# davidfischinger/haf_grasping

Hardware: AMD Instinct MI355X
Metric: grid-cell x rotation SVM evals/sec (higher is better)
Workload: dtype f16

## Files before the change

### haf_grasping_amd/build.py

```python
import os
import re
import subprocess
import sys

HERE = os.path.dirname(os.path.abspath(__file__))
CSRC = os.path.join(HERE, "csrc")
LIB = os.path.join(HERE, "libhafgrasp.so")
LIB_TESTING = os.path.join(HERE, "libhafgrasp_testing.so")
ENGINE_SOURCES = ["engine.cpp", "engine_tables.cpp", "engine_request.cpp", "engine_geometry.cpp", "engine_debug.cpp", "engine_topgrasps.cpp", "engine_graspmap.cpp", "engine_roi.cpp", "engine_depthfilter.cpp", "engine_segment.cpp", "engine_cellsegment.cpp", "engine_plane.cpp", "engine_clearance.cpp", "engine_opening.cpp", "engine_space.cpp", "engine_labelshape.cpp", "engine_objects.cpp", "engine_transfer.cpp", "engine_stage.cpp"]
TESTING_ONLY = ["engine_testing.cpp", "testkernels.hip"]
SOURCES = ["prestages.hip", "features.hip", "contraction.hip", "screen.hip", "recheck.hip", "exact8.hip", "vote.hip", "prob.hip", "topgrasps.hip", "frames.hip", "graspmap.hip", "roi.hip", "depthfilter.hip", "segment.hip", "cellsegment.hip", "plane.hip", "clearance.hip", "opening.hip", "space.hip", "labelshape.hip", "transfer.hip"] + \
          ENGINE_SOURCES + ["parsers.cpp", "model_tables.cpp", "frames_host.cpp", "frame_stage.cpp", "graspmap_host.cpp", "roi_host.cpp", "depthfilter_host.cpp", "segment_host.cpp", "cellsegment_host.cpp", "plane_host.cpp", "clearance_host.cpp", "opening_host.cpp", "space_host.cpp", "labelshape_host.cpp", "transfer_host.cpp", "multi.cpp"]
EXTRA = {"screen.hip": ["-fno-slp-vectorize"]}
HEADERS = ["kernels.h", "device_common.h", "feature_device.h", "screen_band.h", "screen_finish.h", "parsers.h", "model_tables.h", "decq.h", "engine_internal.h", "engine_state.h", "frame_points.h", "frames.h", "frame_stage.h", "frame_group.h", "object_group.h", "label_group.h", "grasp_cells.h", "pick_rules.h", "depth_filter.h", "segment_rules.h", "cell_segment_rules.h", "wave_union.h", "plane_rules.h", "clearance_rules.h", "opening_rules.h", "space_rules.h", "grasp_lane.h", "label_shape.h", "transfer_rules.h"] + TESTING_ONLY + [ os.path.join("..", "..", "include", "hafgrasp.h"),
           os.path.join("..", "cli", "haf_grasp_cli.cpp"), os.path.join("..", "..", "ros_shim", "shim_core.h")]
FLAGS = ["--offload-arch=gfx950", "-O3", "-std=c++17", "-fPIC", "-ffp-contract=off", "-fno-fast-math",
         "-Wall", "-Wno-unused-result", "-Wno-inline-asm"]
ROCM = os.environ.get("ROCM_PATH", "/opt/rocm")
OBJDUMP = os.path.join(ROCM, "lib", "llvm", "bin", "llvm-objdump")
EXP_HAZARD_KERNELS = ["k_svm_screen", "k_svm_rbf_h", "k_svm_rbf"]
EXP_MIN_DISTANCE = 8


def up_to_date():
    if not (os.path.exists(LIB) and os.path.exists(LIB_TESTING)):
        return False
    t = min(os.path.getmtime(LIB), os.path.getmtime(LIB_TESTING))
    deps = [os.path.join(CSRC, f) for f in SOURCES + HEADERS] + [os.path.abspath(__file__)]
    return all(os.path.getmtime(d) <= t for d in deps if os.path.exists(d))
# ... 310 lines not shown

def _compile_and_link(out_lib, out_testing, obj_dir, extra_flags=(), verbose=False, checks=True):
    hipcc = os.environ.get("HIPCC", os.path.join(ROCM, "bin", "hipcc"))
    os.makedirs(obj_dir, exist_ok=True)

    def compile_one(src, suffix="", defs=()):
        obj = os.path.join(obj_dir, os.path.splitext(src)[0] + suffix + ".o")
        cmd = [hipcc] + FLAGS + EXTRA.get(src, []) + os.environ.get("HAF_EXPERIMENT_FLAGS", "").split() + list(extra_flags) + list(defs) + \
              ["-c", os.path.join(CSRC, src), "-o", obj]
        if verbose:
            print(" ".join(cmd))
        subprocess.check_call(cmd)
        return obj

    from concurrent.futures import ThreadPoolExecutor
    jobs = [(src, "", ()) for src in SOURCES] + [(src, "_testing", ("-DHAF_TESTING",)) for src in ENGINE_SOURCES + TESTING_ONLY]
    with ThreadPoolExecutor(max_workers=max(1, int(os.environ.get("HAF_BUILD_JOBS", "4")))) as pool:
        done = list(pool.map(lambda j: compile_one(*j), jobs))
    objs = dict(zip(SOURCES, done[:len(SOURCES)]))
    testing_objs = dict(zip(ENGINE_SOURCES + TESTING_ONLY, done[len(SOURCES):]))
    link = [hipcc, "--offload-arch=gfx950", "-shared", "-fPIC"]
    libs = ["-L" + os.path.join(ROCM, "lib"), "-lrccl", "-lpthread", "-Wl,-rpath," + os.path.join(ROCM, "lib")]
    staged = []
    try:
        for out in (out_lib, out_testing):
            tmp = out + ".unchecked"
            if out == out_lib:
                members = [objs[s] for s in SOURCES]
            else:
                members = [testing_objs.get(s, objs[s]) for s in SOURCES] + [testing_objs[s] for s in TESTING_ONLY]
            cmd = link + members + libs + ["-o", tmp]
            if verbose:
                print(" ".join(cmd))
            subprocess.check_call(cmd)
            staged.append((tmp, out))
# ... 46 lines not shown
```

### haf_grasping_amd/capi.py

```python
import ctypes as C
import os

import numpy as np

HERE = os.path.dirname(os.path.abspath(__file__))
LIB_PATH = os.environ.get("HAF_LIB", os.path.join(HERE, "libhafgrasp.so"))
TESTLIB_PATH = os.environ.get("HAF_TESTLIB", os.path.join(HERE, "libhafgrasp_testing.so"))

HAF_OK, HAF_E_ARG, HAF_E_IO, HAF_E_DEVICE, HAF_E_CAPACITY, HAF_E_BUDGET, HAF_E_INTERNAL = 0, -1, -2, -3, -4, -5, -6
FLAG_KEEP_DEBUG, FLAG_PROFILE, FLAG_FP32_MFMA, FLAG_SPLIT_F16, FLAG_PROBABILITY, FLAG_FULL_RANK = 1, 2, 4, 8, 16, 32
DBG_HEIGHTS, DBG_INTEGRAL, DBG_MASK, DBG_LABELS, DBG_DECISION, DBG_TRANSFORM, DBG_SCREEN_MARGIN, DBG_PROBABILITY, DBG_GRASPSGRID, DBG_ROI = range(10)
SHARD_ROLLS, SHARD_CLOUDS = 0, 1
FRAME_DEPTH_U16, FRAME_DEPTH_F32, FRAME_XYZ_F32 = 0, 1, 2
MAP_NO_CELL = -32768
MAX_LABELS = 4096
STAGES = ["upload", "bin", "integral", "mask", "features", "svm", "refine", "recheck", "vote", "download"]


class Config(C.Structure):
    _fields_ = [("feature_file", C.c_char_p), ("range_file", C.c_char_p), ("model_file", C.c_char_p),
                ("nr_features_without_shaf", C.c_int32), ("grid_h", C.c_int32), ("grid_w", C.c_int32),
                ("n_rolls", C.c_int32), ("roll_step_deg", C.c_int32), ("z_shift", C.c_float),
                ("graspval_top", C.c_int32), ("device", C.c_int32), ("max_clouds", C.c_int32),
                ("max_points", C.c_int64), ("flags", C.c_uint32), ("graspval_th", C.c_int32),
# ... 354 lines not shown
    if testing:
        L.haf_test_decq_host.restype = C.c_double
        L.haf_test_decq_host.argtypes = [C.c_double, C.c_int]
        L.haf_test_scale_host.restype = C.c_double
        L.haf_test_scale_host.argtypes = [C.c_double] * 5
        L.haf_test_sigma_upper.restype = C.c_double
        L.haf_test_sigma_upper.argtypes = [C.c_void_p, C.c_int, C.c_int]
        L.haf_test_table_digest.argtypes = [E, C.c_char_p, C.c_int]
        L.haf_test_host_table_digest.argtypes = [C.POINTER(Config), C.c_double, C.c_double, C.c_char_p, C.c_int, C.c_char_p, C.c_int]
        L.haf_test_decq4_scr.restype = C.c_double
        L.haf_test_decq4_scr.argtypes = [C.c_float]
        L.haf_test_decq4_scr_n.argtypes = [C.c_void_p, C.c_void_p, C.c_int]
        L.haf_test_host_slot_table.argtypes = [C.POINTER(Config), C.c_double, C.c_double, C.c_int] + [C.c_void_p] * 8 + \
            [C.POINTER(C.c_int), C.c_char_p, C.c_int]
        L.haf_test_feature_thresholds.argtypes = [C.c_void_p]
        L.haf_test_feature_form.argtypes = [E, C.c_void_p, C.c_void_p, C.c_void_p, C.c_int, C.POINTER(C.c_int)]
        L.haf_test_screen_finish.argtypes = [E, C.c_void_p, C.c_int, C.c_void_p, C.c_void_p]
        L.haf_test_split3.restype = C.c_double
        L.haf_test_split3.argtypes = [C.c_double, C.c_void_p]
        L.haf_test_decq_device.argtypes = [C.c_void_p, C.c_void_p, C.c_int, C.c_int]
        L.haf_test_mfma_accum.argtypes = [C.c_void_p, C.c_void_p, C.c_void_p, C.c_void_p, C.c_int]
        L.haf_test_mfma_rate.argtypes = [C.c_int, C.c_int, C.POINTER(C.c_double)]
        L.haf_test_mfma_model.argtypes = [C.c_int, C.c_int, C.c_int, C.POINTER(C.c_double)]
        L.haf_test_scale_device.argtypes = [C.c_void_p, C.c_void_p, C.c_void_p, C.c_double, C.c_double, C.c_void_p,
                                            C.c_int]
        L.haf_test_feature_table.argtypes = [C.c_char_p, C.POINTER(C.c_int), C.c_void_p, C.c_void_p, C.c_int]
        L.haf_test_range_table.argtypes = [C.c_char_p, C.POINTER(C.c_double), C.POINTER(C.c_double),
                                           C.POINTER(C.c_int), C.c_void_p, C.c_void_p, C.c_void_p, C.c_int]
        L.haf_test_model.argtypes = [C.c_char_p, C.POINTER(C.c_double), C.POINTER(C.c_double), C.POINTER(C.c_int),
                                     C.POINTER(C.c_int), C.c_void_p, C.c_void_p, C.c_void_p, C.c_void_p, C.c_long]
# ... 1215 lines not shown
```

### haf_grasping_amd/csrc/engine_request.cpp

```cpp
#include "engine_state.h"

namespace haf_host {

static double host_kernel_value(const SvmModel &m, const double *xg, int n, int kx)
{
    double acc = 0.0;
    if (m.kernel_type == HAF_KERNEL_RBF) {
        for (int k = 0; k < kx; k++) {
            const double sv = k < m.dim ? m.sv[(size_t)n * m.dim + k] : 0.0;
            const double dd = xg[(size_t)k * 16] - sv;
            acc += dd * dd;
        }
        return std::exp(-m.gamma * acc);
    }
    for (int k = 0; k < kx; k++) {
        const double sv = k < m.dim ? m.sv[(size_t)n * m.dim + k] : 0.0;
        acc += xg[(size_t)k * 16] * sv;
    }
    if (m.kernel_type == HAF_KERNEL_POLY) {
        double tmp = m.gamma * acc + m.coef0, ret = 1.0;
        for (int t = m.degree; t > 0; t /= 2) { if (t % 2 == 1) ret *= tmp; tmp = tmp * tmp; }
        return ret;
    }
    if (m.kernel_type == HAF_KERNEL_SIGMOID) return std::tanh(m.gamma * acc + m.coef0);
// ... 589 lines not shown

static void fp64_window(haf_engine *e, const Request &q, const TierPlan &p, int off)
{
    if (p.fp64 == FP64_SMALL)
        launch_small_direct(e->d_ii.p, e->d_evalcell.p, e->d_counters.p, e->mdl.fd.p, e->mdl.sv64.p, e->mdl.exact, q.d, e->flag_cap, e->d_dec_exact.p,
                            e->d_labels.p, list_buf(e, p.fp64_out), e->list_cap, nullptr, q.s, list_buf(e, p.fp64_in), list_counter(p.fp64_in), off);
    else
        launch_recheck_mfma(e->d_ii.p, e->d_evalcell.p, e->mdl.fd.p, e->mdl.sv64.p, e->mdl.exact, list_buf(e, p.fp64_in), e->flag_cap, off, e->d_counters.p,
                            e->d_x64.p, e->d_part64.p, p.i8 ? e->d_dec_exacti.p : e->d_dec_exact.p, e->d_labels.p, list_buf(e, p.fp64_out), e->list_cap,
                            q.d, q.s, nullptr, false, list_counter(p.fp64_in), e->d_tier_words.p);
}
static void i8_window(haf_engine *e, const Request &q, const TierPlan &p, int off)
{
    launch_recheck_i8(e->d_ii.p, e->d_evalcell.p, e->mdl.fd.p, e->mdl.sv_i8.p, e->mdl.i8, e->range.lower, e->range.upper, list_buf(e, p.i8_in), e->flag_cap,
                      off, e->d_counters.p, e->d_x64.p, e->d_part64.p, e->d_dec_exact.p, e->d_labels.p, list_buf(e, p.i8_out), e->list_cap, q.d, q.s,
                      e->d_tier_words.p);
}

static int vote_and_wait(haf_engine *e, const Request &q)
{
    const hipStream_t s = q.s;
    mark(e, HAF_ST_VOTE);
    if (q.from.roi)
        launch_vote_roi(e->d_labels.p, reinterpret_cast<const float *>(e->d_heights.p), e->d_brcount.p, e->d_ev16.p, e->d_topkey.p, e->d_rowmax.p,
                        e->d_rec.p, e->d_roi_cells.p, q.d, s);
    else
        launch_vote(e->d_labels.p, reinterpret_cast<const float *>(e->d_heights.p), e->d_brcount.p, e->d_ev16.p, e->d_topkey.p, e->d_rowmax.p, e->d_rec.p, q.d, s);
    mark(e, HAF_ST_DOWNLOAD);
    HIPCHK(e, hipMemcpyAsync(e->out_block.host, e->out_block.dev.p, kCntBytes + (size_t)q.B * q.R * sizeof(RollRecordDev), hipMemcpyDeviceToHost, s));
    mark(e, HAF_ST_COUNT);
    if (q.short_request) {
// ... 298 lines not shown
```

### haf_grasping_amd/csrc/engine_tables.cpp

```cpp
#include "engine_state.h"

namespace haf_host {

TableSwitches table_switches()
{
    TableSwitches s;
    s.no_cr = test_env("HAF_NO_CR") != nullptr;
    s.no_lr = test_env("HAF_NO_LR") != nullptr;
    s.cr_no_centre = test_env("HAF_CR_NO_CENTRE") != nullptr;
    s.no_cr_t1 = test_env("HAF_NO_CR_T1") != nullptr;
    s.no_i8 = test_env("HAF_NO_I8") != nullptr;
    s.no_fast_groups = test_env("HAF_NO_FAST_GROUPS") != nullptr;
    s.screen_no_centre = test_env("HAF_SCREEN_NO_CENTRE") != nullptr;
    s.lr_unfused = test_env("HAF_LR_UNFUSED") != nullptr;
    s.no_lr_plain = test_env("HAF_NO_LR_PLAIN") != nullptr;
    s.kappa_t1_measured = test_env("HAF_KAPPA_T1_MEASURED") != nullptr;
    s.prob_host_all = test_env("HAF_PROB_HOST_ALL") != nullptr;
    s.host_exp_all = test_env("HAF_HOST_EXP_ALL") != nullptr;
    if (const char *g = test_env("HAF_GUARD_REL")) { s.guard_rel_set = true; s.guard_rel = guard_knob(g); }
    if (const char *g = test_env("HAF_GUARD0_REL")) { s.guard0_rel_set = true; s.guard0_rel = guard_knob(g); }
    if (const char *g = test_env("HAF_GUARD2_REL")) { s.guard2_rel_set = true; s.guard2_rel = guard_knob(g); }
    if (const char *g = test_env("HAF_GUARD_I8_REL")) { s.guard_i8_rel_set = true; s.guard_i8_rel = guard_knob(g); }
    return s;
}

static TableInputs table_inputs(const haf_engine *e)
{
    TableInputs in;
    in.cfg = e->cfg;
// ... 158 lines not shown
```

### haf_grasping_amd/csrc/engine_testing.cpp

```cpp
#include "engine_state.h"
#include "screen_finish.h"
#include "screen_band.h"

#ifndef HAF_TESTING
#error "engine_testing.cpp belongs to the testing build (-DHAF_TESTING)"
#endif

namespace haf_host {
namespace {
struct CanaryRec { char *user; size_t bytes; const char *file; int line; };
std::mutex g_canary_mu;
std::vector<CanaryRec> g_canary;
}
void canary_register(void *user, size_t bytes, const char *file, int line)
{
    std::lock_guard<std::mutex> lk(g_canary_mu);
    g_canary.push_back(CanaryRec{static_cast<char *>(user), bytes, file, line});
}
void canary_unregister(void *user)
{
    std::lock_guard<std::mutex> lk(g_canary_mu);
    for (size_t i = 0; i < g_canary.size(); i++)
        if (g_canary[i].user == user) { g_canary[i] = g_canary.back(); g_canary.pop_back(); return; }
}
// ... 597 lines not shown
                lr_finish_band(r, lb, o[0], o[1], o[2], o[3]);
            }
        }
        return (int)HAF_OK;
    });
    return rc == HAF_E_INTERNAL ? say(rc) : rc;
}

int haf_test_feature_thresholds(long long *out3)
{
    if (!out3) return HAF_E_ARG;
    out3[0] = kSmallEvals; out3[1] = kWaves16Evals; out3[2] = kLargeEvals;
    return HAF_OK;
}

int haf_test_feature_form(haf_engine *e, int *form, int *flags, unsigned long long *iiabs, int cap, int *n)
{
    if (!e || !form) return HAF_E_ARG;
    form[0] = e->feature_form; form[1] = e->feature_sp_kind; form[2] = e->feature_sp.cr_poly;
    const int br = e->last.B * e->last.R;
    if (n) *n = br;
    if (!flags && !iiabs) return HAF_OK;
    if (br <= 0 || br > cap) return HAF_E_ARG;
    if (hipDeviceSynchronize() != hipSuccess) return HAF_E_DEVICE;
    if (flags && (!e->d_inexact.p || (size_t)br > e->d_inexact.n ||
                  hipMemcpy(flags, e->d_inexact.p, (size_t)br * sizeof(int), hipMemcpyDeviceToHost) != hipSuccess)) return HAF_E_DEVICE;
    if (iiabs && (!e->d_iiabs.p || (size_t)br > e->d_iiabs.n ||
                  hipMemcpy(iiabs, e->d_iiabs.p, (size_t)br * sizeof(unsigned long long), hipMemcpyDeviceToHost) != hipSuccess)) return HAF_E_DEVICE;
    return HAF_OK;
}
// ... 224 lines not shown
```

### haf_grasping_amd/csrc/exact8.hip

```cpp
#include "device_common.h"

namespace haf {

typedef int i32x4 __attribute__((ext_vector_type(4)));

constexpr int kI8Waves = 4;
constexpr int kI8Evals = 16 * kI8Waves;
constexpr int kI8Split = 8;
static_assert(kRecheckPartRows == 2 * kI8Split + 1, "part64 layout shared with the fp64 tier");
constexpr int kI8TileLoads = kI8GroupBytes / (256 * 16);
static_assert(kI8TileLoads * 256 * 16 == kI8GroupBytes, "tile image = whole 16-byte loads of 256 threads");

__device__ __forceinline__ int window_count8(int total, int off, int cap) { return max(0, min(total - off, cap)); }

__device__ __forceinline__ double exp2_poly(double y)
{
    const double n = rint(y);
    const double f = y - n;
    double p = 4.4455382718708101e-10;
    p = fma(p, f, 7.0549116208011209e-09);
    p = fma(p, f, 1.0178086009239696e-07);
    p = fma(p, f, 1.3215486790144305e-06);
    p = fma(p, f, 1.5252733804059838e-05);
    p = fma(p, f, 0.00015403530393381606);
    p = fma(p, f, 0.0013333558146428441);
    p = fma(p, f, 0.0096181291076284769);
    p = fma(p, f, 0.055504108664821576);
    p = fma(p, f, 0.24022650695910069);
    p = fma(p, f, 0.69314718055994529);
    p = fma(p, f, 1.0);
    return ldexp(p, (int)fmax(n, -1200.0));
}

__device__ __forceinline__ void i8_tile_mfma(const char *bt, int lane, const i32x4 (&a)[kI8Slices][kI8Steps], i32x4 (&acc)[5])
{
#pragma unroll
    for (int w = 0; w < 5; w++) acc[w] = i32x4{0, 0, 0, 0};
    i32x4 b[kI8Slices], bn[kI8Slices];
#pragma unroll
    for (int k = 0; k < kI8Slices; k++) b[k] = *reinterpret_cast<const i32x4 *>(bt + (k * kI8Steps) * 1024 + lane * 16);
#pragma unroll
    for (int ks = 0; ks < kI8Steps; ks++) {
        if (ks + 1 < kI8Steps) {
#pragma unroll
            for (int k = 0; k < kI8Slices; k++) bn[k] = *reinterpret_cast<const i32x4 *>(bt + (k * kI8Steps + ks + 1) * 1024 + lane * 16);
        }
#define HAF_I8_MFMA(j, k) acc[(j) + (k)] = __builtin_amdgcn_mfma_i32_16x16x64_i8(a[j][ks], b[k], acc[(j) + (k)], 0, 0, 0)
        HAF_I8_MFMA(0, 3); HAF_I8_MFMA(1, 3); HAF_I8_MFMA(0, 2); HAF_I8_MFMA(1, 2); HAF_I8_MFMA(0, 1); HAF_I8_MFMA(2, 2); HAF_I8_MFMA(2, 1);
        HAF_I8_MFMA(1, 1); HAF_I8_MFMA(0, 0); HAF_I8_MFMA(3, 0); HAF_I8_MFMA(3, 1); HAF_I8_MFMA(2, 0); HAF_I8_MFMA(1, 0);
#undef HAF_I8_MFMA
#pragma unroll
        for (int k = 0; k < kI8Slices; k++) b[k] = bn[k];
    }
}

__device__ __forceinline__ void i8_tile_epilogue(const i32x4 (&acc)[5], const double (&xx)[4], double ss, double cf, double gamma2, double dq_scale,
                                                 double (&part)[4], double (&pabs)[4])
{
#pragma unroll
    for (int r = 0; r < 4; r++) {
        const int u1 = (acc[1][r] << 7) + acc[2][r], u2 = (acc[3][r] << 7) + acc[4][r];
        const double dq = fma(fma((double)acc[0][r], 16384.0, (double)u1), 16384.0, (double)u2);
        const double d2 = fma(dq_scale, dq, xx[r] + ss);
        const double kv = exp2_poly(-gamma2 * d2);
        part[r] = fma(cf, kv, part[r]);
        pabs[r] = fma(fabs(cf), kv, pabs[r]);
    }
}

__device__ __forceinline__ void i8_split(int n_flag, int flag_cap, int n_tiles, int &splits, size_t &pitch)
{
    const bool fine = (long)n_flag * 4 <= (long)flag_cap && n_tiles >= 16 * kI8Split && flag_cap >= 4 && n_flag <= 1024;
    const int n_groups = (n_flag + kI8Evals - 1) / kI8Evals;
    splits = fine ? max(kI8Split, min(4 * kI8Split, 512 / max(n_groups, 1))) : kI8Split;
    pitch = fine ? (size_t)(flag_cap / 4) : (size_t)flag_cap;
}

__global__ __launch_bounds__(256, 2) void k_recheck_i8(const char *__restrict__ ximg, const char *__restrict__ svimg, I8Params p,
                                                       int flag_cap, int list_off, const int *__restrict__ counters, int cslot,
                                                       double *__restrict__ part64)
{
    __shared__ __attribute__((aligned(16))) char bt[kI8SvTileBytes];
    const int n_flag = window_count8(counters[cslot], list_off, flag_cap);
    const int n_groups = (n_flag + kI8Evals - 1) / kI8Evals;
    const int tid = threadIdx.x, wave = tid >> 6, lane = tid & 63;
    const int n_tiles = p.n_sv_pad / 16;
    int splits;
    size_t pitch;
    i8_split(n_flag, flag_cap, n_tiles, splits, pitch);
    const int tiles_per_part = (n_tiles + splits - 1) / splits;
    const double *xnorm = part64 + (size_t)(2 * kI8Split) * flag_cap;
    for (int task = blockIdx.x; task < n_groups * splits; task += gridDim.x) {
        const int g = task / splits, h = task - g * splits;
// ... 83 lines not shown
            v += __shfl_xor(v, 1, 64); w += __shfl_xor(w, 1, 64);
            part[r] = v; pabs[r] = w;
        }
        if ((lane & 15) == 0) {
#pragma unroll
            for (int r = 0; r < 4; r++) {
                const int sl = grp * 16 + 4 * (lane >> 4) + r;
                if (sl < n_flag) {
                    part64[(size_t)(2 * h) * pitch + sl] = part[r];
                    part64[(size_t)(2 * h + 1) * pitch + sl] = pabs[r];
                }
            }
        }
    }
}

__global__ __launch_bounds__(256) void k_recheck_i8_combine(const double *__restrict__ part64, const int *__restrict__ evalcell, I8Params p,
                                                            const int *__restrict__ flag_list, int flag_cap, int list_off,
                                                            int *__restrict__ counters, int cslot, double *__restrict__ dec_exact,
                                                            int8_t *__restrict__ labels, int *__restrict__ flagi_list, int flagi_cap,
                                                            unsigned long long *__restrict__ words)
{
    const int n_flag = window_count8(counters[cslot], list_off, flag_cap);
    const int lane = threadIdx.x & 63;
    int splits;
    size_t pitch;
    i8_split(n_flag, flag_cap, p.n_sv_pad / 16, splits, pitch);
    for (int base = blockIdx.x * 256 + (threadIdx.x & ~63); base < n_flag; base += gridDim.x * 256) {
        const int sl = base + lane;
        bool undecided = false;
// ... 25 lines not shown
            if (lane == 0) words[base >> 6] = bal;
        }
    }
}

__global__ __launch_bounds__(kListCompactThreads) void k_i8_handover(const unsigned long long *__restrict__ words, const int *__restrict__ flag_list,
                                                                     int flag_cap, int list_off, int *__restrict__ counters, int cslot,
                                                                     int *__restrict__ flagi_list, int flagi_cap)
{
    __shared__ int s_scan[kListCompactThreads];
    list_compact_body(words, window_count8(counters[cslot], list_off, flag_cap), flag_list, flagi_list, flagi_cap, counters, CNT_FLAGGEDI, s_scan);
}

void launch_recheck_i8(const float *ii, const int *evalcell, const FeatDesc *fd, const void *sv_i8, I8Params p, double lower, double upper,
                       const int *flag_list, int window_cap, int list_off, int *counters, void *ximg, double *part64, double *dec_exact,
                       int8_t *labels, int *flagi_list, int flagi_cap, Dims d, hipStream_t s, unsigned long long *words)
{
    const int groups = (window_cap + kI8Evals - 1) / kI8Evals;
    if (groups <= 0) return;
    flag_list += list_off;
    dec_exact += list_off;
    launch_features(ii, evalcell, counters, fd, reinterpret_cast<float *>(ximg), reinterpret_cast<float *>(part64 + (size_t)(2 * kI8Split) * window_cap),
                    d, lower, upper, 0.0f, window_cap, XMODE_I8, ScreenParams{}, flag_list, CNT_FLAGGED, window_cap, false, window_cap, nullptr,
                    nullptr, s, list_off);
    const long tasks = (long)groups * 4 * kI8Split;
    hipLaunchKernelGGL(k_recheck_i8, dim3((unsigned)(tasks < 8192 ? tasks : 8192)), dim3(256), 0, s, (const char *)ximg, (const char *)sv_i8, p,
                       window_cap, list_off, counters, CNT_FLAGGED, part64);
    const int blocks = groups < 2048 ? groups : 2048;
    hipLaunchKernelGGL(k_recheck_i8_combine, dim3(blocks), dim3(256), 0, s, part64, evalcell, p, flag_list, window_cap, list_off, counters,
                       CNT_FLAGGED, dec_exact, labels, flagi_list, flagi_cap, words);
    if (words) hipLaunchKernelGGL(k_i8_handover, dim3(1), dim3(kListCompactThreads), 0, s, words, flag_list, window_cap, list_off, counters, CNT_FLAGGED,
                                  flagi_list, flagi_cap);
}

}
```

### haf_grasping_amd/csrc/kernels.h

```cpp
#pragma once

#include <hip/hip_runtime.h>
#include <stddef.h>
#include <stdint.h>
#include "frame_points.h"
#include "frames.h"
#include "grasp_cells.h"
#include "pick_rules.h"

namespace haf {

constexpr int kKP = 324;
constexpr int kKSteps = kKP / 2;
constexpr int kDP = 328;
constexpr int kTile = 32;
constexpr int kTileFloats = kDP * kTile;
constexpr int kSvmBlockEvals = 256;
constexpr int kSvmThreads = 512;
constexpr int kHListParts = 4;

constexpr int kHK = 336;
constexpr int kHFull = 10;
constexpr int kHSteps = kHK / 16;
constexpr int kHMatBytes = kHSteps * 1024;
// ... 211 lines not shown
enum { CNT_EVALS = 0, CNT_FLAGGED = 1, CNT_ERROR = 2, CNT_FLAGGED2 = 3, CNT_FLAGGED0 = 4,
       CNT_INEXACT = 5,
       CNT_FLAGGEDI = 6,
       CNT_FLAGGED0B = 7,
       CNT_BYPASS = 8,
       CNT_T1_N = 9,
       CNT_T1_ADD = 10,
       CNT_COUNT = 12 };

constexpr int kI8Q = 23;
constexpr long kI8Max = 63L * (2097152L + 16384L + 128L + 1L);
constexpr int kI8Slices = 4;
constexpr int kI8Steps = 6;
constexpr int kI8GroupBytes = kI8Slices * kI8Steps * 1024;
constexpr int kI8SvTileBytes = kI8GroupBytes + 256;
struct I8Params {
    double gamma, rho;
    double gamma2;
    double drop;
    double delta;
    double dq_scale;
    double s_max;
    double guard_scale;
    int n_sv_pad, gv0, gv1, pad;
};
void launch_recheck_i8(const float *ii, const int *evalcell, const FeatDesc *fd, const void *sv_i8, I8Params p, double lower, double upper,
                       const int *flag_list, int window_cap, int list_off, int *counters, void *ximg, double *part64, double *dec_exact,
                       int8_t *labels, int *flagi_list, int flagi_cap, Dims d, hipStream_t s,
                       unsigned long long *words = nullptr);

constexpr int kM64Rows = 326;

struct RollRecordDev { int vote; short row, col; float h_locmax; int n_evals; };

struct ProbParams {
    double A, B;
    int gv0, gv1;
    float hdr;
    int host_all;
    double dec_slack;
};
void launch_probability_eval(const double *dec_exact, const int *evalcell, const int *counters, ProbParams P, int8_t *labels, float *own,
                             double *ptext, int *near_list, int near_cap, int *counters_rw, long evals_cap, hipStream_t s);
void launch_prob_list(int *counters, int slot, int *list, int cap, hipStream_t s);
// ... 286 lines not shown
```

### haf_grasping_amd/csrc/model_tables.cpp

```cpp
#include "model_tables.h"

#include <algorithm>
#include <cmath>
#include <cstdio>
#include <cstdlib>
#include <cstring>

namespace haf_host {

float header_grid_value(int label0, int label1)
{
    char line[96];
    snprintf(line, sizeof line, "labels %d %d", label0, label1);
    const std::string ln(line);
    const int res = (int)atof(ln.substr(0, 2).c_str());
    int start = (int)ln.find(" ", 0), end = (int)ln.find(" ", (size_t)start + 1);
    if (res > 0) { start = end; end = (int)ln.find(" ", (size_t)start + 1); }
    const float prob = (float)atof(ln.substr((size_t)start, (size_t)end).c_str());
    return res * prob;
}

int label_grid_value(int label)
{
    char buf[32];
// ... 1031 lines not shown
        sv64[(size_t)kKP * t.n_sv_pad + n] = ss;
        sv64[(size_t)(kKP + 1) * t.n_sv_pad + n] = m.coef[(size_t)n];
        coef64[(size_t)n] = m.coef[(size_t)n];
        ss_max = std::max(ss_max, ss);
    }
    return ss_max;
}

void int8_planes(Work &w)
{
    const haf_config &c = w.in.cfg;
    const SvmModel &m = *w.in.model;
    const TableSwitches &sw = w.in.sw;
    ModelTables &t = w.t;
    t.i8_active = !(c.flags & HAF_FLAG_PROBABILITY) && !sw.no_i8 && t.kx <= 64 * kI8Steps && !w.in.generic_kernel;
    if (!t.i8_active) return;
    const int n_tiles16 = t.n_sv_pad / 16;
    std::vector<char> img((size_t)n_tiles16 * kI8SvTileBytes, 0);
    double s_max2 = 0.0;
    double sv_abs_max = 0.0;
    for (int n = 0; n < m.n_sv; n++)
        for (int k = 0; k < m.dim; k++) sv_abs_max = std::max(sv_abs_max, std::fabs(m.sv[(size_t)n * m.dim + k]));
    int qs = kI8Q;
    while (qs < 30 && (sv_abs_max * std::ldexp(1.0, qs + 1) + 1.0) <= (double)kI8Max) qs++;
    if (!(sv_abs_max < 1e30)) t.i8_active = false;
    for (int n = 0; n < m.n_sv && t.i8_active; n++) {
        char *tile = img.data() + (size_t)(n / 16) * kI8SvTileBytes;
        const int col = n % 16;
        long long ssq = 0;
        for (int k = 0; k < m.dim; k++) {
// ... 132 lines not shown
```

### haf_grasping_amd/csrc/model_tables.h

```cpp
#pragma once
#include "../../include/hafgrasp.h"
#include "kernels.h"
#include "parsers.h"

#include <string>
#include <vector>

using namespace haf;

namespace haf_host {

enum { MODE_SCREEN = 0, MODE_SPLIT = 1, MODE_F32 = 2 };
inline int contraction_mode(const haf_config &c)
{
    if (c.flags & HAF_FLAG_FP32_MFMA) return MODE_F32;
    if (c.flags & HAF_FLAG_SPLIT_F16) return MODE_SPLIT;
    return MODE_SCREEN;
}

struct TableSwitches {
    bool no_cr = false;
    bool no_lr = false;
    bool cr_no_centre = false;
    bool no_cr_t1 = false;
    bool no_i8 = false;
    bool no_fast_groups = false;
    bool screen_no_centre = false;
    bool lr_unfused = false;
    bool no_lr_plain = false;
    bool kappa_t1_measured = false;
    bool prob_host_all = false;
    bool host_exp_all = false;
    bool guard_rel_set = false, guard0_rel_set = false, guard2_rel_set = false, guard_i8_rel_set = false;
    double guard_rel = 1.0, guard0_rel = 1.0, guard2_rel = 1.0, guard_i8_rel = 1.0;
};

struct TableInputs {
    haf_config cfg{};
    const std::vector<FeatureRow> *features = nullptr;
    const RangeTable *range = nullptr;
    const SvmModel *model = nullptr;
    double mfma_kappa = 12.0, mfma_kappa16 = 12.0;
    bool generic_kernel = false;
// ... 47 lines not shown
    I8Params i8{};
    ProbParams prob{};

    int nf = 0, kx = 0, n_sv_tiles = 0, sv_tile_neg = 0, n_sv_pad = 0;
    double sum_abs_coef = 0;
    bool screen_active = true;
    bool cr_available = false;
    bool lr_available = false;
    bool lr_fused = true;
    bool lr_plain_available = false;
    bool t1_cr_available = false, i8_active = false;
    int lr_rank = 0;
    int gv0 = 0, gv1 = 0;
    bool prob_mode = false;
    double host_exp_thr = 0.0;
};

template <class T> using HostBuf = std::vector<T>;
struct ModelTables : TableSet<HostBuf>, ModelConsts {
    std::vector<int> slot_rep;
    std::vector<double> slot_mu;
};

struct TableError {
    int code = HAF_OK;
    std::string msg;
};

TableError build_model_tables(const TableInputs &in, ModelTables &t);

// ... 6 lines not shown
```

### haf_grasping_amd/csrc/screen.hip

```cpp
#include "kernels.h"
#include "screen_band.h"
#include <algorithm>
#include <cmath>
#include <vector>

namespace haf {

typedef float f32x4 __attribute__((ext_vector_type(4)));
typedef _Float16 half8 __attribute__((ext_vector_type(8)));
typedef _Float16 half4 __attribute__((ext_vector_type(4)));

__device__ __forceinline__ void dma_piece(const char *gbase, unsigned lds_dst, unsigned lane16)
{
    asm volatile("s_mov_b32 m0, %0\n\ts_nop 0\n\tglobal_load_lds_dwordx4 %1, %2" ::"s"(lds_dst), "v"(lane16), "s"(gbase) : "memory", "m0");
}

struct TileDma {
    const char *g[kS0WavePieces];
    unsigned l[kS0WavePieces];
};
__device__ __forceinline__ TileDma tile_dma(const char *gtile, unsigned lds_slot, const int (&poff)[kS0WavePieces])
{
    TileDma d;
#pragma unroll
    for (int q = 0; q < kS0WavePieces; q++) { d.g[q] = gtile + poff[q]; d.l[q] = lds_slot + (unsigned)poff[q]; }
    return d;
}
__device__ __forceinline__ void stage_sv_tile_s0(const TileDma &d, unsigned lane16)
{
    asm volatile("s_nop 4");
// ... 1127 lines not shown
```

Baseline: 535.3 million.

## Pipeline int8 recheck kernel with LDS DMA ring and interleaved epilogue

Rewrites the exact int8 recheck kernel so support-vector tiles are streamed into an LDS ring buffer through direct global-to-LDS loads. Each tile's MFMA sequence is interleaved with the DMA issues for the next tile and with the previous tile's double-precision exp epilogue, using sched barriers. The goal is to hide global load latency and epilogue ALU time behind matrix work. The old staged kernel is kept only as a testing-build option, and the grid cap becomes configurable, at the cost of more LDS per workgroup and more complex scheduling.

```diff
diff --git a/haf_grasping_amd/build.py b/haf_grasping_amd/build.py
--- a/haf_grasping_amd/build.py
+++ b/haf_grasping_amd/build.py
@@ -9,10 +9,11 @@
 LIB_TESTING = os.path.join(HERE, "libhafgrasp_testing.so")
 ENGINE_SOURCES = ["engine.cpp", "engine_tables.cpp", "engine_request.cpp", "engine_geometry.cpp", "engine_debug.cpp", "engine_topgrasps.cpp", "engine_graspmap.cpp", "engine_roi.cpp", "engine_depthfilter.cpp", "engine_segment.cpp", "engine_cellsegment.cpp", "engine_plane.cpp", "engine_clearance.cpp", "engine_opening.cpp", "engine_space.cpp", "engine_labelshape.cpp", "engine_objects.cpp", "engine_transfer.cpp", "engine_stage.cpp"]
 TESTING_ONLY = ["engine_testing.cpp", "testkernels.hip"]
+TESTING_KERNELS = ["exact8.hip"]
 SOURCES = ["prestages.hip", "features.hip", "contraction.hip", "screen.hip", "recheck.hip", "exact8.hip", "vote.hip", "prob.hip", "topgrasps.hip", "frames.hip", "graspmap.hip", "roi.hip", "depthfilter.hip", "segment.hip", "cellsegment.hip", "plane.hip", "clearance.hip", "opening.hip", "space.hip", "labelshape.hip", "transfer.hip"] + \
           ENGINE_SOURCES + ["parsers.cpp", "model_tables.cpp", "frames_host.cpp", "frame_stage.cpp", "graspmap_host.cpp", "roi_host.cpp", "depthfilter_host.cpp", "segment_host.cpp", "cellsegment_host.cpp", "plane_host.cpp", "clearance_host.cpp", "opening_host.cpp", "space_host.cpp", "labelshape_host.cpp", "transfer_host.cpp", "multi.cpp"]
 EXTRA = {"screen.hip": ["-fno-slp-vectorize"]}
-HEADERS = ["kernels.h", "device_common.h", "feature_device.h", "screen_band.h", "screen_finish.h", "parsers.h", "model_tables.h", "decq.h", "engine_internal.h", "engine_state.h", "frame_points.h", "frames.h", "frame_stage.h", "frame_group.h", "object_group.h", "label_group.h", "grasp_cells.h", "pick_rules.h", "depth_filter.h", "segment_rules.h", "cell_segment_rules.h", "wave_union.h", "plane_rules.h", "clearance_rules.h", "opening_rules.h", "space_rules.h", "grasp_lane.h", "label_shape.h", "transfer_rules.h"] + TESTING_ONLY + [ os.path.join("..", "..", "include", "hafgrasp.h"),
+HEADERS = ["kernels.h", "device_common.h", "lds_dma.h", "feature_device.h", "screen_band.h", "screen_finish.h", "parsers.h", "model_tables.h", "decq.h", "engine_internal.h", "engine_state.h", "frame_points.h", "frames.h", "frame_stage.h", "frame_group.h", "object_group.h", "label_group.h", "grasp_cells.h", "pick_rules.h", "depth_filter.h", "segment_rules.h", "cell_segment_rules.h", "wave_union.h", "plane_rules.h", "clearance_rules.h", "opening_rules.h", "space_rules.h", "grasp_lane.h", "label_shape.h", "transfer_rules.h"] + TESTING_ONLY + [ os.path.join("..", "..", "include", "hafgrasp.h"),
            os.path.join("..", "cli", "haf_grasp_cli.cpp"), os.path.join("..", "..", "ros_shim", "shim_core.h")]
 FLAGS = ["--offload-arch=gfx950", "-O3", "-std=c++17", "-fPIC", "-ffp-contract=off", "-fno-fast-math",
          "-Wall", "-Wno-unused-result", "-Wno-inline-asm"]
@@ -353,11 +354,11 @@
         return obj
 
     from concurrent.futures import ThreadPoolExecutor
-    jobs = [(src, "", ()) for src in SOURCES] + [(src, "_testing", ("-DHAF_TESTING",)) for src in ENGINE_SOURCES + TESTING_ONLY]
+    jobs = [(src, "", ()) for src in SOURCES] + [(src, "_testing", ("-DHAF_TESTING",)) for src in ENGINE_SOURCES + TESTING_KERNELS + TESTING_ONLY]
     with ThreadPoolExecutor(max_workers=max(1, int(os.environ.get("HAF_BUILD_JOBS", "4")))) as pool:
         done = list(pool.map(lambda j: compile_one(*j), jobs))
     objs = dict(zip(SOURCES, done[:len(SOURCES)]))
-    testing_objs = dict(zip(ENGINE_SOURCES + TESTING_ONLY, done[len(SOURCES):]))
+    testing_objs = dict(zip(ENGINE_SOURCES + TESTING_KERNELS + TESTING_ONLY, done[len(SOURCES):]))
     link = [hipcc, "--offload-arch=gfx950", "-shared", "-fPIC"]
     libs = ["-L" + os.path.join(ROCM, "lib"), "-lrccl", "-lpthread", "-Wl,-rpath," + os.path.join(ROCM, "lib")]
     staged = []
diff --git a/haf_grasping_amd/capi.py b/haf_grasping_amd/capi.py
--- a/haf_grasping_amd/capi.py
+++ b/haf_grasping_amd/capi.py
@@ -392,6 +392,7 @@
         L.haf_test_host_slot_table.argtypes = [C.POINTER(Config), C.c_double, C.c_double, C.c_int] + [C.c_void_p] * 8 + \
             [C.POINTER(C.c_int), C.c_char_p, C.c_int]
         L.haf_test_feature_thresholds.argtypes = [C.c_void_p]
+        L.haf_test_exact_ring.argtypes = [C.c_void_p]
         L.haf_test_feature_form.argtypes = [E, C.c_void_p, C.c_void_p, C.c_void_p, C.c_int, C.POINTER(C.c_int)]
         L.haf_test_screen_finish.argtypes = [E, C.c_void_p, C.c_int, C.c_void_p, C.c_void_p]
         L.haf_test_split3.restype = C.c_double
diff --git a/haf_grasping_amd/csrc/engine_request.cpp b/haf_grasping_amd/csrc/engine_request.cpp
--- a/haf_grasping_amd/csrc/engine_request.cpp
+++ b/haf_grasping_amd/csrc/engine_request.cpp
@@ -627,7 +627,7 @@
 {
     launch_recheck_i8(e->d_ii.p, e->d_evalcell.p, e->mdl.fd.p, e->mdl.sv_i8.p, e->mdl.i8, e->range.lower, e->range.upper, list_buf(e, p.i8_in), e->flag_cap,
                       off, e->d_counters.p, e->d_x64.p, e->d_part64.p, e->d_dec_exact.p, e->d_labels.p, list_buf(e, p.i8_out), e->list_cap, q.d, q.s,
-                      e->d_tier_words.p);
+                      e->d_tier_words.p, e->mdl.i8_staged, e->mdl.i8_grid);
 }
 
 static int vote_and_wait(haf_engine *e, const Request &q)
diff --git a/haf_grasping_amd/csrc/engine_tables.cpp b/haf_grasping_amd/csrc/engine_tables.cpp
--- a/haf_grasping_amd/csrc/engine_tables.cpp
+++ b/haf_grasping_amd/csrc/engine_tables.cpp
@@ -13,6 +13,8 @@
     s.no_fast_groups = test_env("HAF_NO_FAST_GROUPS") != nullptr;
     s.screen_no_centre = test_env("HAF_SCREEN_NO_CENTRE") != nullptr;
     s.lr_unfused = test_env("HAF_LR_UNFUSED") != nullptr;
+    s.i8_staged = test_env("HAF_I8_STAGED") != nullptr;
+    if (const char *v = test_env("HAF_I8_GRID")) s.i8_grid = std::max(1, atoi(v));
     s.no_lr_plain = test_env("HAF_NO_LR_PLAIN") != nullptr;
     s.kappa_t1_measured = test_env("HAF_KAPPA_T1_MEASURED") != nullptr;
     s.prob_host_all = test_env("HAF_PROB_HOST_ALL") != nullptr;
diff --git a/haf_grasping_amd/csrc/engine_testing.cpp b/haf_grasping_amd/csrc/engine_testing.cpp
--- a/haf_grasping_amd/csrc/engine_testing.cpp
+++ b/haf_grasping_amd/csrc/engine_testing.cpp
@@ -635,6 +635,14 @@
     return HAF_OK;
 }
 
+int haf_test_exact_ring(long long *out8)
+{
+    if (!out8) return HAF_E_ARG;
+    out8[0] = kI8SvTileBytes; out8[1] = kI8GroupBytes; out8[2] = kI8Ring; out8[3] = kI8RingBytes; out8[4] = kI8WavePieces;
+    out8[5] = kI8RingWaves; out8[6] = kI8WgsPerCu; out8[7] = kCuLdsBytes;
+    return HAF_OK;
+}
+
 int haf_test_feature_form(haf_engine *e, int *form, int *flags, unsigned long long *iiabs, int cap, int *n)
 {
     if (!e || !form) return HAF_E_ARG;
diff --git a/haf_grasping_amd/csrc/exact8.hip b/haf_grasping_amd/csrc/exact8.hip
--- a/haf_grasping_amd/csrc/exact8.hip
+++ b/haf_grasping_amd/csrc/exact8.hip
@@ -1,4 +1,5 @@
 #include "device_common.h"
+#include "lds_dma.h"
 
 namespace haf {
 
@@ -32,6 +33,117 @@
     return ldexp(p, (int)fmax(n, -1200.0));
 }
 
+constexpr int i8_pair_j(int q) { constexpr int J[13] = {0, 1, 0, 1, 0, 2, 2, 1, 0, 3, 3, 2, 1}; return J[q]; }
+constexpr int i8_pair_k(int q) { constexpr int K[13] = {3, 3, 2, 2, 1, 2, 1, 1, 0, 0, 1, 0, 0}; return K[q]; }
+constexpr int kI8TileMfmas = 13 * kI8Steps;
+constexpr int kI8EpiOps = 28;
+constexpr int kI8EpiSteps = 4 * kI8EpiOps;
+constexpr int kI8EpiSlots = kI8TileMfmas - kI8WavePieces;
+
+struct I8TileDma {
+    const char *g[kI8WavePieces];
+    unsigned l[kI8WavePieces];
+};
+__device__ __forceinline__ I8TileDma i8_tile_dma(const char *gtile, unsigned lds_slot, const int (&poff)[kI8WavePieces])
+{
+    I8TileDma d;
+#pragma unroll
+    for (int q = 0; q < kI8WavePieces; q++) { d.g[q] = gtile + poff[q]; d.l[q] = lds_slot + (unsigned)poff[q]; }
+    return d;
+}
+
+struct I8Epi {
+    int u1[4], u2[4], ni[4];
+    double d0[4], d1[4], d2[4], y[4], n[4], f[4], p[4];
+};
+template <int STEP>
+__device__ __forceinline__ void i8_epi_op(I8Epi &e, const i32x4 (&acc)[5], const double (&xx)[4], double ss, double cf, double gamma2,
+                                          double dq_scale, double (&part)[4], double (&pabs)[4])
+{
+    constexpr int r = STEP & 3;
+    switch (STEP >> 2) {
+    case 0: e.u1[r] = (acc[1][r] << 7) + acc[2][r]; break;
+    case 1: e.u2[r] = (acc[3][r] << 7) + acc[4][r]; break;
+    case 2: e.d0[r] = (double)acc[0][r]; break;
+    case 3: e.d1[r] = (double)e.u1[r]; break;
+    case 4: e.d2[r] = (double)e.u2[r]; break;
+    case 5: e.d0[r] = fma(e.d0[r], 16384.0, e.d1[r]); break;
+    case 6: e.d0[r] = fma(e.d0[r], 16384.0, e.d2[r]); break;
+    case 7: e.d1[r] = xx[r] + ss; break;
+    case 8: e.d0[r] = fma(dq_scale, e.d0[r], e.d1[r]); break;
+    case 9: e.y[r] = -gamma2 * e.d0[r]; break;
+    case 10: e.n[r] = rint(e.y[r]); break;
+    case 11: e.f[r] = e.y[r] - e.n[r]; break;
+    case 12: e.p[r] = fma(4.4455382718708101e-10, e.f[r], 7.0549116208011209e-09); break;
+    case 13: e.p[r] = fma(e.p[r], e.f[r], 1.0178086009239696e-07); break;
+    case 14: e.p[r] = fma(e.p[r], e.f[r], 1.3215486790144305e-06); break;
+    case 15: e.p[r] = fma(e.p[r], e.f[r], 1.5252733804059838e-05); break;
+    case 16: e.p[r] = fma(e.p[r], e.f[r], 0.00015403530393381606); break;
+    case 17: e.p[r] = fma(e.p[r], e.f[r], 0.0013333558146428441); break;
+    case 18: e.p[r] = fma(e.p[r], e.f[r], 0.0096181291076284769); break;
+    case 19: e.p[r] = fma(e.p[r], e.f[r], 0.055504108664821576); break;
+    case 20: e.p[r] = fma(e.p[r], e.f[r], 0.24022650695910069); break;
+    case 21: e.p[r] = fma(e.p[r], e.f[r], 0.69314718055994529); break;
+    case 22: e.p[r] = fma(e.p[r], e.f[r], 1.0); break;
+    case 23: e.n[r] = fmax(e.n[r], -1200.0); break;
+    case 24: e.ni[r] = (int)e.n[r]; break;
+    case 25: e.p[r] = ldexp(e.p[r], e.ni[r]); break;
+    case 26: part[r] = fma(cf, e.p[r], part[r]); break;
+    default: pabs[r] = fma(fabs(cf), e.p[r], pabs[r]); break;
+    }
+}
+
+#define HAF_I8_SB() __builtin_amdgcn_sched_barrier(0)
+template <bool EPI, int M>
+__device__ __forceinline__ void i8_tile_step(const char *bl, const i32x4 (&a)[kI8Slices][kI8Steps], i32x4 (&acc)[5], const i32x4 (&old)[5],
+                                             const double (&xx)[4], double ss, double cf, double gamma2, double dq_scale, double (&part)[4],
+                                             double (&pabs)[4], const I8TileDma &dma, unsigned lane16, I8Epi &e, i32x4 (&b)[kI8Slices],
+                                             i32x4 (&bn)[kI8Slices])
+{
+    constexpr int ks = M / 13, q = M % 13, j = i8_pair_j(q), k = i8_pair_k(q), w = j + k;
+    if constexpr (q == 0 && ks + 1 < kI8Steps) {
+#pragma unroll
+        for (int kk = 0; kk < kI8Slices; kk++) bn[kk] = *reinterpret_cast<const i32x4 *>(bl + (kk * kI8Steps + ks + 1) * 1024);
+        HAF_I8_SB();
+    }
+    constexpr bool first = ks == 0 && q == (w == 0 ? 8 : w == 1 ? 4 : w == 2 ? 2 : w == 3 ? 0 : 1);
+    if constexpr (first) acc[w] = __builtin_amdgcn_mfma_i32_16x16x64_i8(a[j][ks], b[k], i32x4{0, 0, 0, 0}, 0, 0, 0);
+    else acc[w] = __builtin_amdgcn_mfma_i32_16x16x64_i8(a[j][ks], b[k], acc[w], 0, 0, 0);
+    HAF_I8_SB();
+    if constexpr (M < kI8WavePieces) {
+        dma_piece(dma.g[M], dma.l[M], lane16);
+        HAF_I8_SB();
+    } else if constexpr (EPI) {
+        constexpr int s0 = (M - kI8WavePieces) * kI8EpiSteps / kI8EpiSlots, s1 = (M - kI8WavePieces + 1) * kI8EpiSteps / kI8EpiSlots;
+        static_assert(s1 - s0 <= 2, "one or two epilogue instructions behind an MFMA");
+        if constexpr (s0 < s1) { i8_epi_op<s0>(e, old, xx, ss, cf, gamma2, dq_scale, part, pabs); HAF_I8_SB(); }
+        if constexpr (s0 + 1 < s1) { i8_epi_op<s0 + 1>(e, old, xx, ss, cf, gamma2, dq_scale, part, pabs); HAF_I8_SB(); }
+    }
+    if constexpr (q == 12) {
+#pragma unroll
+        for (int kk = 0; kk < kI8Slices; kk++) b[kk] = bn[kk];
+    }
+    if constexpr (M + 1 < kI8TileMfmas)
+        i8_tile_step<EPI, M + 1>(bl, a, acc, old, xx, ss, cf, gamma2, dq_scale, part, pabs, dma, lane16, e, b, bn);
+}
+
+template <bool EPI>
+__device__ __forceinline__ void i8_tile_body(const char *cur, int lane, const i32x4 (&a)[kI8Slices][kI8Steps], i32x4 (&acc)[5],
+                                             const i32x4 (&old)[5], const double (&xx)[4], double ss, double cf, double gamma2, double dq_scale,
+                                             double (&part)[4], double (&pabs)[4], const I8TileDma &dma, unsigned lane16)
+{
+    const char *bl = cur + lane * 16;
+    HAF_I8_SB();
+    I8Epi e;
+    i32x4 b[kI8Slices], bn[kI8Slices];
+#pragma unroll
+    for (int k = 0; k < kI8Slices; k++) b[k] = *reinterpret_cast<const i32x4 *>(bl + (k * kI8Steps) * 1024);
+    HAF_I8_SB();
+    i8_tile_step<EPI, 0>(bl, a, acc, old, xx, ss, cf, gamma2, dq_scale, part, pabs, dma, lane16, e, b, bn);
+}
+#undef HAF_I8_SB
+
+#ifdef HAF_TESTING
 __device__ __forceinline__ void i8_tile_mfma(const char *bt, int lane, const i32x4 (&a)[kI8Slices][kI8Steps], i32x4 (&acc)[5])
 {
 #pragma unroll
@@ -53,6 +165,7 @@
         for (int k = 0; k < kI8Slices; k++) b[k] = bn[k];
     }
 }
+#endif
 
 __device__ __forceinline__ void i8_tile_epilogue(const i32x4 (&acc)[5], const double (&xx)[4], double ss, double cf, double gamma2, double dq_scale,
                                                  double (&part)[4], double (&pabs)[4])
@@ -76,7 +189,126 @@
     pitch = fine ? (size_t)(flag_cap / 4) : (size_t)flag_cap;
 }
 
-__global__ __launch_bounds__(256, 2) void k_recheck_i8(const char *__restrict__ ximg, const char *__restrict__ svimg, I8Params p,
+__global__ __launch_bounds__(256, kI8WgsPerCu) void k_recheck_i8(const char *__restrict__ ximg, const char *__restrict__ svimg, I8Params p,
+                                                                 int flag_cap, int list_off, const int *__restrict__ counters, int cslot,
+                                                                 double *__restrict__ part64)
+{
+    __shared__ __attribute__((aligned(16))) char ring[kI8RingBytes];
+    const int n_flag = window_count8(counters[cslot], list_off, flag_cap);
+    const int n_groups = (n_flag + kI8Evals - 1) / kI8Evals;
+    const int tid = threadIdx.x, wave = tid >> 6, lane = tid & 63;
+    const int n_tiles = p.n_sv_pad / 16;
+    int splits;
+    size_t pitch;
+    i8_split(n_flag, flag_cap, n_tiles, splits, pitch);
+    splits = __builtin_amdgcn_readfirstlane(splits);
+    const int tiles_per_part = __builtin_amdgcn_readfirstlane((n_tiles + splits - 1) / splits);
+    const double *xnorm = part64 + (size_t)(2 * kI8Split) * flag_cap;
+    const unsigned lds0 = (unsigned)(uintptr_t)ring;
+    const unsigned lane16 = (unsigned)lane * 16u, lane4 = (unsigned)lane * 4u;
+    const int wave_u = __builtin_amdgcn_readfirstlane(wave);
+    int poff[kI8WavePieces];
+#pragma unroll
+    for (int q = 0; q < kI8WavePieces; q++) poff[q] = (wave_u + kI8RingWaves * q) * 1024;
+    static_assert(kI8Waves == kI8RingWaves, "one share of the pieces per wave");
+    constexpr int kAhead = kI8Ring - 1;
+    for (int task = blockIdx.x; task < n_groups * splits; task += gridDim.x) {
+        const int g = __builtin_amdgcn_readfirstlane(task / splits), h = task - g * splits;
+        const int t_begin = h * tiles_per_part, t_end = min(n_tiles, t_begin + tiles_per_part);
+        const int grp = g * kI8Waves + wave;
+        __syncthreads();
+        if (t_begin < t_end) {
+            asm volatile("s_nop 4");
+#pragma unroll
+            for (int i = 0; i < kAhead; i++) {
+                if (t_begin + i < t_end) {
+                    const char *gt = svimg + (size_t)(t_begin + i) * kI8SvTileBytes;
+                    const I8TileDma d0 = i8_tile_dma(gt, lds0 + i * kI8SvTileBytes, poff);
+#pragma unroll
+                    for (int q = 0; q < kI8WavePieces; q++) dma_piece(d0.g[q], d0.l[q], lane16);
+                    if (wave_u == 0) dma_piece_256(gt + kI8GroupBytes, lds0 + i * kI8SvTileBytes + kI8GroupBytes, lane4);
+                }
+            }
+        }
+        i32x4 a[kI8Slices][kI8Steps];
+        {
+            const char *xg = ximg + (size_t)grp * kI8GroupBytes + lane * 16;
+#pragma unroll
+            for (int j = 0; j < kI8Slices; j++)
+#pragma unroll
+                for (int ks = 0; ks < kI8Steps; ks++) a[j][ks] = *reinterpret_cast<const i32x4 *>(xg + (j * kI8Steps + ks) * 1024);
+        }
+        double xx[4];
+#pragma unroll
+        for (int r = 0; r < 4; r++) {
+            const int sl = grp * 16 + 4 * (lane >> 4) + r;
+            xx[r] = (sl < n_flag) ? xnorm[sl] : 0.0;
+        }
+#pragma unroll
+        for (int j = 0; j < kI8Slices; j++)
+#pragma unroll
+            for (int ks = 0; ks < kI8Steps; ks++) asm volatile("" : "+v"(a[j][ks]));
+#pragma unroll
+        for (int r = 0; r < 4; r++) asm volatile("" : "+v"(xx[r]));
+        asm volatile("s_waitcnt vmcnt(0)" ::: "memory");
+        __syncthreads();
+        double part[4] = {0, 0, 0, 0}, pabs[4] = {0, 0, 0, 0};
+        i32x4 acc_prev[5], acc_cur[5];
+#pragma unroll
+        for (int w = 0; w < 5; w++) acc_prev[w] = i32x4{0, 0, 0, 0};
+        double ss_prev = 0.0, cf_prev = 0.0;
+        int slot = 0, slot_n = kAhead % kI8Ring;
+#define HAF_I8_TILE(EPI, t)                                                                                                            \
+        {                                                                                                                                  \
+            const char *cur = ring + slot * kI8SvTileBytes;                                                                                \
+            const int tn = (t) + kAhead < t_end ? (t) + kAhead : t_begin;                                                                  \
+            const char *gt = svimg + (size_t)tn * kI8SvTileBytes;                                                                          \
+            const unsigned ls = lds0 + (unsigned)(slot_n * kI8SvTileBytes);                                                                \
+            const I8TileDma dma = i8_tile_dma(gt, ls, poff);                                                                               \
+            if (wave_u == 0) dma_piece_256(gt + kI8GroupBytes, ls + kI8GroupBytes, lane4);                                                 \
+                \
+                                                                   \
+            const double *cst = reinterpret_cast<const double *>(cur + kI8GroupBytes);                                                     \
+            const double ss_cur = cst[lane & 15], cf_cur = cst[16 + (lane & 15)];                                                          \
+            i8_tile_body<EPI>(cur, lane, a, acc_cur, acc_prev, xx, ss_prev, cf_prev, p.gamma2, p.dq_scale, part, pabs, dma, lane16);       \
+            ss_prev = ss_cur; cf_prev = cf_cur;                                                                                            \
+            _Pragma("unroll") for (int w = 0; w < 5; w++) acc_prev[w] = acc_cur[w];                                                        \
+            slot = slot + 1 == kI8Ring ? 0 : slot + 1;                                                                                     \
+            slot_n = slot_n + 1 == kI8Ring ? 0 : slot_n + 1;                                                                               \
+            asm volatile("s_waitcnt vmcnt(0)" ::: "memory");                                                                               \
+            __builtin_amdgcn_s_barrier();                                                                                                  \
+            asm volatile("" ::: "memory");                                    \
+        }
+        if (t_begin < t_end) {
+            HAF_I8_TILE(false, t_begin);
+            for (int t = t_begin + 1; t < t_end; t++) HAF_I8_TILE(true, t);
+            i8_tile_epilogue(acc_prev, xx, ss_prev, cf_prev, p.gamma2, p.dq_scale, part, pabs);
+        }
+#undef HAF_I8_TILE
+#pragma unroll
+        for (int r = 0; r < 4; r++) {
+            double v = part[r], w = pabs[r];
+            v += __shfl_xor(v, 8, 64); w += __shfl_xor(w, 8, 64);
+            v += __shfl_xor(v, 4, 64); w += __shfl_xor(w, 4, 64);
+            v += __shfl_xor(v, 2, 64); w += __shfl_xor(w, 2, 64);
+            v += __shfl_xor(v, 1, 64); w += __shfl_xor(w, 1, 64);
+            part[r] = v; pabs[r] = w;
+        }
+        if ((lane & 15) == 0) {
+#pragma unroll
+            for (int r = 0; r < 4; r++) {
+                const int sl = grp * 16 + 4 * (lane >> 4) + r;
+                if (sl < n_flag) {
+                    part64[(size_t)(2 * h) * pitch + sl] = part[r];
+                    part64[(size_t)(2 * h + 1) * pitch + sl] = pabs[r];
+                }
+            }
+        }
+    }
+}
+
+#ifdef HAF_TESTING
+__global__ __launch_bounds__(256, 2) void k_recheck_i8_staged(const char *__restrict__ ximg, const char *__restrict__ svimg, I8Params p,
                                                        int flag_cap, int list_off, const int *__restrict__ counters, int cslot,
                                                        double *__restrict__ part64)
 {
@@ -190,6 +422,7 @@
         }
     }
 }
+#endif
 
 __global__ __launch_bounds__(256) void k_recheck_i8_combine(const double *__restrict__ part64, const int *__restrict__ evalcell, I8Params p,
                                                             const int *__restrict__ flag_list, int flag_cap, int list_off,
@@ -245,7 +478,7 @@
 
 void launch_recheck_i8(const float *ii, const int *evalcell, const FeatDesc *fd, const void *sv_i8, I8Params p, double lower, double upper,
                        const int *flag_list, int window_cap, int list_off, int *counters, void *ximg, double *part64, double *dec_exact,
-                       int8_t *labels, int *flagi_list, int flagi_cap, Dims d, hipStream_t s, unsigned long long *words)
+                       int8_t *labels, int *flagi_list, int flagi_cap, Dims d, hipStream_t s, unsigned long long *words, bool staged, int grid_cap)
 {
     const int groups = (window_cap + kI8Evals - 1) / kI8Evals;
     if (groups <= 0) return;
@@ -255,8 +488,16 @@
                     d, lower, upper, 0.0f, window_cap, XMODE_I8, ScreenParams{}, flag_list, CNT_FLAGGED, window_cap, false, window_cap, nullptr,
                     nullptr, s, list_off);
     const long tasks = (long)groups * 4 * kI8Split;
-    hipLaunchKernelGGL(k_recheck_i8, dim3((unsigned)(tasks < 8192 ? tasks : 8192)), dim3(256), 0, s, (const char *)ximg, (const char *)sv_i8, p,
-                       window_cap, list_off, counters, CNT_FLAGGED, part64);
+    const long cap = grid_cap > 0 ? grid_cap : 8192;
+    const dim3 grid((unsigned)(tasks < cap ? tasks : cap));
+#ifdef HAF_TESTING
+    if (staged) hipLaunchKernelGGL(k_recheck_i8_staged, grid, dim3(256), 0, s, (const char *)ximg, (const char *)sv_i8, p, window_cap, list_off,
+                                   counters, CNT_FLAGGED, part64);
+    else
+#endif
+    hipLaunchKernelGGL(k_recheck_i8, grid, dim3(256), 0, s, (const char *)ximg, (const char *)sv_i8, p, window_cap, list_off, counters,
+                       CNT_FLAGGED, part64);
+    (void)staged;
     const int blocks = groups < 2048 ? groups : 2048;
     hipLaunchKernelGGL(k_recheck_i8_combine, dim3(blocks), dim3(256), 0, s, part64, evalcell, p, flag_list, window_cap, list_off, counters,
                        CNT_FLAGGED, dec_exact, labels, flagi_list, flagi_cap, words);
diff --git a/haf_grasping_amd/csrc/kernels.h b/haf_grasping_amd/csrc/kernels.h
--- a/haf_grasping_amd/csrc/kernels.h
+++ b/haf_grasping_amd/csrc/kernels.h
@@ -249,6 +249,18 @@
 constexpr int kI8Steps = 6;
 constexpr int kI8GroupBytes = kI8Slices * kI8Steps * 1024;
 constexpr int kI8SvTileBytes = kI8GroupBytes + 256;
+#ifndef HAF_I8_RING
+#define HAF_I8_RING 2
+#endif
+constexpr int kI8Ring = HAF_I8_RING;
+constexpr int kI8RingWaves = 4;
+constexpr int kI8WavePieces = kI8GroupBytes / (kI8RingWaves * 1024);
+constexpr int kI8RingBytes = kI8Ring * kI8SvTileBytes;
+constexpr int kI8WgsPerCu = 2;
+constexpr int kCuLdsBytes = 160 * 1024;
+static_assert(kI8Ring == 2 || kI8Ring == 3, "a double or a triple buffer");
+static_assert(kI8WavePieces * kI8RingWaves * 1024 == kI8GroupBytes, "the digit image = whole 1 KiB pieces, the same number per wave");
+static_assert(kI8SvTileBytes % 16 == 0 && kI8WgsPerCu * kI8RingBytes <= kCuLdsBytes, "two workgroups' rings fit a CU's LDS");
 struct I8Params {
     double gamma, rho;
     double gamma2;
@@ -262,7 +274,8 @@
 void launch_recheck_i8(const float *ii, const int *evalcell, const FeatDesc *fd, const void *sv_i8, I8Params p, double lower, double upper,
                        const int *flag_list, int window_cap, int list_off, int *counters, void *ximg, double *part64, double *dec_exact,
                        int8_t *labels, int *flagi_list, int flagi_cap, Dims d, hipStream_t s,
-                       unsigned long long *words = nullptr);
+                       unsigned long long *words = nullptr,
+                       bool staged = false, int grid_cap = 0);
 
 constexpr int kM64Rows = 326;
 
diff --git a/haf_grasping_amd/csrc/lds_dma.h b/haf_grasping_amd/csrc/lds_dma.h
--- /dev/null
+++ b/haf_grasping_amd/csrc/lds_dma.h
@@ -0,0 +1,15 @@
+#pragma once
+
+namespace haf {
+
+__device__ __forceinline__ void dma_piece(const char *gbase, unsigned lds_dst, unsigned lane16)
+{
+    asm volatile("s_mov_b32 m0, %0\n\ts_nop 0\n\tglobal_load_lds_dwordx4 %1, %2" ::"s"(lds_dst), "v"(lane16), "s"(gbase) : "memory", "m0");
+}
+
+__device__ __forceinline__ void dma_piece_256(const char *gbase, unsigned lds_dst, unsigned lane4)
+{
+    asm volatile("s_mov_b32 m0, %0\n\ts_nop 0\n\tglobal_load_lds_dword %1, %2" ::"s"(lds_dst), "v"(lane4), "s"(gbase) : "memory", "m0");
+}
+
+}
diff --git a/haf_grasping_amd/csrc/model_tables.cpp b/haf_grasping_amd/csrc/model_tables.cpp
--- a/haf_grasping_amd/csrc/model_tables.cpp
+++ b/haf_grasping_amd/csrc/model_tables.cpp
@@ -1069,6 +1069,8 @@
     const TableSwitches &sw = w.in.sw;
     ModelTables &t = w.t;
     t.i8_active = !(c.flags & HAF_FLAG_PROBABILITY) && !sw.no_i8 && t.kx <= 64 * kI8Steps && !w.in.generic_kernel;
+    t.i8_staged = sw.i8_staged;
+    t.i8_grid = sw.i8_grid;
     if (!t.i8_active) return;
     const int n_tiles16 = t.n_sv_pad / 16;
     std::vector<char> img((size_t)n_tiles16 * kI8SvTileBytes, 0);
diff --git a/haf_grasping_amd/csrc/model_tables.h b/haf_grasping_amd/csrc/model_tables.h
--- a/haf_grasping_amd/csrc/model_tables.h
+++ b/haf_grasping_amd/csrc/model_tables.h
@@ -27,6 +27,8 @@
     bool no_fast_groups = false;
     bool screen_no_centre = false;
     bool lr_unfused = false;
+    bool i8_staged = false;
+    int i8_grid = 0;
     bool no_lr_plain = false;
     bool kappa_t1_measured = false;
     bool prob_host_all = false;
@@ -104,6 +106,8 @@
     int gv0 = 0, gv1 = 0;
     bool prob_mode = false;
     double host_exp_thr = 0.0;
+    bool i8_staged = false;
+    int i8_grid = 0;
 };
 
 template <class T> using HostBuf = std::vector<T>;
diff --git a/haf_grasping_amd/csrc/screen.hip b/haf_grasping_amd/csrc/screen.hip
--- a/haf_grasping_amd/csrc/screen.hip
+++ b/haf_grasping_amd/csrc/screen.hip
@@ -1,4 +1,5 @@
 #include "kernels.h"
+#include "lds_dma.h"
 #include "screen_band.h"
 #include <algorithm>
 #include <cmath>
@@ -9,11 +10,6 @@
 typedef float f32x4 __attribute__((ext_vector_type(4)));
 typedef _Float16 half8 __attribute__((ext_vector_type(8)));
 typedef _Float16 half4 __attribute__((ext_vector_type(4)));
-
-__device__ __forceinline__ void dma_piece(const char *gbase, unsigned lds_dst, unsigned lane16)
-{
-    asm volatile("s_mov_b32 m0, %0\n\ts_nop 0\n\tglobal_load_lds_dwordx4 %1, %2" ::"s"(lds_dst), "v"(lane16), "s"(gbase) : "memory", "m0");
-}
 
 struct TileDma {
     const char *g[kS0WavePieces];
```

Result: no change. 537.6 million (median of 3 runs) (+0.4%).
